# GATB/dsk

Measured on AMD Instinct MI355X. Metric: distinct k-mers counted/sec (whole node), k=31, higher is better.
Workload: dtype u64

## Files before the change

dsk_amd/csrc/dskgpu.hip:

```cpp
#include <algorithm>
#include <cstdio>
#include <cstring>
#include <cstdlib>
#include <cmath>
#include <string>
#include <vector>

#include <thread>
#include <system_error>
#include "engine.h"
#include "kernels.h"
#include "superkmer_recv.h"
#include "rawparse.h"

#include <rocprim/device/device_radix_sort.hpp>

#define DSKGPU_VERSION "dskgpu 0.1 (gfx950)"

namespace {

thread_local std::string g_create_err;

__global__ __launch_bounds__(1024) void k_place_probe(unsigned long long* __restrict__ out, unsigned long long n) {
    const unsigned long long per_block = n / gridDim.x, per_stream = per_block / 512;
    unsigned long long* base = out + (unsigned long long)blockIdx.x * per_block;
    const int r = threadIdx.x >> 5, l = threadIdx.x & 31;
    for (unsigned long long off = 0; off + 32 <= per_stream; off += 32)
        for (int p = r; p < 512; p += 32) base[(unsigned long long)p * per_stream + off + l] = off;
}
int g_place_k = -1;
float place_probe_ms(void* p, size_t bytes) {
    hipEvent_t a, b;
    if (hipEventCreate(&a) != hipSuccess || hipEventCreate(&b) != hipSuccess) return 0.f;
    float best = 1e30f;
    for (int i = 0; i < 3; ++i) {
        (void)hipEventRecord(a, 0);
        hipLaunchKernelGGL(k_place_probe, dim3(256), dim3(1024), 0, 0, static_cast<unsigned long long*>(p), (unsigned long long)(bytes / 8));
        (void)hipEventRecord(b, 0);
        (void)hipEventSynchronize(b);
        float ms = 0.f; (void)hipEventElapsedTime(&ms, a, b);
        if (i && ms < best) best = ms;
    }
    (void)hipEventDestroy(a); (void)hipEventDestroy(b);
    return best;
}
}

hipError_t placed_malloc(void** out, size_t bytes) {
    if (g_place_k < 0) { const char* e = getenv("DSKGPU_PLACE"); g_place_k = e ? atoi(e) : 0; }
    size_t free_b = 0, total_b = 0;
    if (g_place_k < 2 || bytes < (size_t(1) << 28) || hipMemGetInfo(&free_b, &total_b) != hipSuccess) return hipMalloc(out, bytes);
    const int K = (int)std::min<size_t>((size_t)g_place_k, free_b / 2 / bytes);
    if (K < 2) return hipMalloc(out, bytes);
    std::vector<void*> cand; std::vector<float> ms;
    for (int i = 0; i < K; ++i) {
        void* q = nullptr;
        if (hipMalloc(&q, bytes) != hipSuccess) { (void)hipGetLastError(); break; }
        static const size_t probe_max = getenv("DSKGPU_PLACE_GB") ? (size_t)(atof(getenv("DSKGPU_PLACE_GB")) * (1ull << 30)) : ~size_t(0);
        cand.push_back(q); ms.push_back(place_probe_ms(q, std::min(bytes, probe_max)));
    }
    if (cand.empty()) return hipErrorOutOfMemory;
    size_t best = 0;
    for (size_t i = 1; i < cand.size(); ++i) if (ms[i] < ms[best]) best = i;
    for (size_t i = 0; i < cand.size(); ++i) if (i != best) (void)hipFree(cand[i]);
// ... 194 lines not shown
template <int W>
inline void launch_count(dskgpu_ctx* ctx, unsigned grid, typename KeyT<W>::T* keys, typename KeyT<W>::T* solid_keys, u32* solid_ab, u32* ovf, const CountParams& cp) {
    launch_count_impl(ctx, grid, keys, solid_keys, solid_ab, ovf, cp);
}

struct Plan {
    int levels;
    u32 P1, P2, F;
    DigitSpec d1, d2;
};

#define TARGET_KEYS 2900
#define TARGET_KEYS2 2560
#ifndef TARGET_KEYS4
#define TARGET_KEYS4 640
#endif
#ifndef OPT_GROUPS4
#define OPT_GROUPS4 OPT_GROUPS
#endif
#define MAX_LEVEL_BINS 2048
#define ONE_LEVEL_BINS 1024
#define CH2 65536u
#define OPT_GROUPS 545u
#define OPT_GROUPS2 1023u
inline u32 opt_groups(int W) { return W == 2 ? (AL_G2 == 8 ? 1022u : OPT_GROUPS2) : (W == 1 && AL_G1 == 16) ? 546u : W == 4 ? OPT_GROUPS4 : OPT_GROUPS; }
inline u64 target_keys(int W) { return W == 1 ? TARGET_KEYS : W == 2 ? TARGET_KEYS2 : TARGET_KEYS4; }
#define OPT_CAP 4360u

bool make_plan(u64 n_upper, int extra_bits, int W, u32 num_cu, Plan* pl) {
    const u64 target = target_keys(W);
    u64 F = ((n_upper + target - 1) / target) << extra_bits;
    if (F < 2) F = 2;
    if (F <= ONE_LEVEL_BINS) { pl->levels = 1; pl->P1 = (u32)F; pl->P2 = 1; }
    else {
        u64 p2max = MAX_LEVEL_BINS; while (p2max > 64 && ascatter_lds(W, (u32)p2max) > 160 * 1024) --p2max;
        u64 p1 = 1; while (p1 * p1 < F) ++p1;
        const bool large = F >= (u64)num_cu * 64;
        if (large) {
            p1 = std::max<u64>((F + p2max - 2) / (p2max - 1), num_cu);
            p1 = (p1 + num_cu - 1) / num_cu * num_cu;
            if (p1 > MAX_LEVEL_BINS - 8) p1 = MAX_LEVEL_BINS - 8;
        }
        u64 p2 = (F + p1 - 1) / p1;
        if (p2 % 2 == 0 && p2 + 1 <= p2max) ++p2;
        if (p1 > MAX_LEVEL_BINS || p2 > MAX_LEVEL_BINS) return false;
        pl->levels = 2; pl->P1 = (u32)p1; pl->P2 = (u32)p2;
    }
    pl->F = pl->P1 * pl->P2;
    pl->d1 = DigitSpec{1u, pl->P1, 0u, 1u, 1u, 0u};
    pl->d2 = DigitSpec{2u, pl->P1, pl->P2, 1u, 1u, 0u};
    return true;
}

void build_descs1(dskgpu_ctx* ctx, u64 n_units_total, u64 tile, u64 max_chunks, u32* nch_out) {
    const u64 ntiles = std::max<u64>(1, (n_units_total + tile - 1) / tile);
    u64 nch = std::min<u64>(ntiles, max_chunks);
    const u64 tpc = (ntiles + nch - 1) / nch;
    nch = (ntiles + tpc - 1) / tpc;
    ctx->h_descs1.resize(nch);
    for (u64 c = 0; c < nch; ++c) {
        ChunkDesc d;
        d.begin = c * tpc * tile;
        d.end = std::min<u64>(n_units_total, (c + 1) * tpc * tile);
        if (d.begin > d.end) d.begin = d.end;
        d.flat_base = (u32)c;
        d.stride = (u32)nch;
        ctx->h_descs1[c] = d;
    }
    *nch_out = (u32)nch;
}

void build_descs1_slices(dskgpu_ctx* ctx, u64 tile, u64 max_chunks, u32* nch_out) {
    const size_t S = ctx->rec_slice_end.size();
    ctx->h_descs1.clear(); ctx->h_slice_chunk.assign(S + 1, 0);
    const u64 per_slice = std::max<u64>(1, max_chunks / S);
    u64 rb = 0;
    for (size_t sl = 0; sl < S; ++sl) {
        const u64 re = ctx->rec_slice_end[sl];
        ctx->h_slice_chunk[sl] = (u32)ctx->h_descs1.size();
        if (re > rb) {
            const u64 ntiles = (re - rb + tile - 1) / tile;
            u64 nch = std::min<u64>(ntiles, per_slice);
            const u64 tpc = (ntiles + nch - 1) / nch;
            nch = (ntiles + tpc - 1) / tpc;
            for (u64 c = 0; c < nch; ++c) {
                ChunkDesc d;
                d.begin = rb + c * tpc * tile; d.end = std::min<u64>(re, rb + (c + 1) * tpc * tile);
                d.flat_base = 0; d.stride = 0;
                ctx->h_descs1.push_back(d);
            }
        }
        rb = re;
    }
    ctx->h_slice_chunk[S] = (u32)ctx->h_descs1.size();
    for (auto& d : ctx->h_descs1) d.stride = (u32)ctx->h_descs1.size();
    *nch_out = (u32)ctx->h_descs1.size();
}

#define REC_RESIZE 1001
int rec_gate_upto(dskgpu_ctx* ctx, u32 upto) {
    if (!ctx->rec_gate) return DSKGPU_OK;
    const u32 n = (u32)ctx->rec_slice_end.size();
    for (; ctx->rec_gated < std::min(upto, n); ++ctx->rec_gated)
        if (ctx->rec_gate(ctx->rec_gate_user, ctx->rec_gated) != 0) ctx->rec_gate_failed = true;
    return ctx->rec_gate_failed ? fail(ctx, DSKGPU_E_STATE, "a slice of the exchange did not arrive (the caller's gate failed)") : DSKGPU_OK;
}
int rec_gate_all(dskgpu_ctx* ctx) { return rec_gate_upto(ctx, 0xFFFFFFFFu); }

int sk_sizes(dskgpu_ctx* ctx, u64* total_out) {
    const u64 nrec = ctx->rec_n; const u32 R = ctx->sender.sp.R;
    { const int e = rec_gate_all(ctx); if (e) return e; }
    u64 nch = std::min<u64>((nrec + SKX_NT - 1) / SKX_NT, (u64)ctx->num_cu * 16);
    u64 rpc = (nrec + nch - 1) / nch;
    rpc = (rpc + SKX_NT - 1) / SKX_NT * SKX_NT;
    nch = (nrec + rpc - 1) / rpc;
    if (rpc * SK_MAXN >= 0xFFFFFFFFull) return fail(ctx, DSKGPU_E_ARG, "too many records per chunk");
    CK(ctx->sk_sums.ensure(nch * 4)); CK(ctx->sk_cbase.ensure(nch * 8));
    ctx->h_sk_sums.assign(nch, 0); ctx->h_sk_cbase.assign(nch, 0);
    hipLaunchKernelGGL(k_sk_count, dim3((unsigned)nch), dim3(SKX_NT), 0, ctx->stream, ctx->rec_src, nrec, R, (u32)rpc, ctx->sk_sums.as<u32>());
    CKL("k_sk_count");
    CK(hipMemcpyAsync(ctx->h_sk_sums.data(), ctx->sk_sums.p, nch * 4, hipMemcpyDeviceToHost, ctx->stream));
    CK(hipStreamSynchronize(ctx->stream));
    u64 total = 0;
    for (u64 c = 0; c < nch; ++c) { ctx->h_sk_cbase[c] = total; total += ctx->h_sk_sums[c]; }
    CK(hipMemcpyAsync(ctx->sk_cbase.p, ctx->h_sk_cbase.data(), nch * 8, hipMemcpyHostToDevice, ctx->stream));
    ctx->rec_nch = nch; ctx->rec_rpc = rpc; ctx->rec_sized = true;
    *total_out = total;
    return DSKGPU_OK;
}

template <int W>
int expand_records(dskgpu_ctx* ctx, u64 total) {
    typedef typename KeyT<W>::T Key;
    if (ctx->rec_expanded) return DSKGPU_OK;
    if (!ctx->rec_sized) {
        u64 real = 0;
        const int e = sk_sizes(ctx, &real);
        if (e) return e;
        if (real != total && ctx->rec_hint_est) { ctx->rec_hint = real; return REC_RESIZE; }
        if (real != total) return fail(ctx, DSKGPU_E_ARG, "dskgpu_mg_count_sized: n_kmers does not match the k-mers inside the records");
    }
    { const int e = rec_gate_all(ctx); if (e) return e; }
    CK(ctx->sk_keys.ensure((total + 1) * sizeof(Key)));
    hipLaunchKernelGGL(k_sk_expand<W>, dim3((unsigned)ctx->rec_nch), dim3(SKX_NT), 0, ctx->stream, ctx->rec_src, ctx->rec_n, ctx->sender.sp.R,
                       (int)ctx->cfg.kmer_size, (u32)ctx->rec_rpc, ctx->sk_cbase.as<u64>(), ctx->sk_keys.as<Key>());
    CKL("k_sk_expand");
    ctx->rec_expanded = true;
    ctx->mark("mg_expand");
// ... 62 lines not shown
        u32 found = 0;
        for (u32 i = 0; i < n;) {
            u32 j = i + 1;
            while (j < n && kk[j] == kk[i]) ++j;
            if ((u64)(j - i) * 20 >= n) { cands.push_back({load[bin] * (double)(j - i) / (double)n, kk[i], bin}); ++found; }
            i = j;
        }
        if (ctx->tune.verbose) fprintf(stderr, "[dskgpu]   bin %u load %.0f: %u keys collected, %u dominant\n", bin, load[bin], n, found);
    }
    std::sort(cands.begin(), cands.end(), [](const Cand& a, const Cand& b) { return a.est > b.est; });
    if (cands.size() > HV_KEYS) cands.resize(HV_KEYS);
    ctx->h_hv_keys.assign((size_t)HV_KEYS * W, DSK_EMPTY);
    for (size_t x = 0; x < cands.size(); ++x) {
        for (int y = 0; y < W; ++y) ctx->h_hv_keys[x * W + y] = cands[x].key.w[y];
        load[cands[x].bin] -= cands[x].est;
    }
    u32 nheavy = (u32)cands.size();
    if (nheavy) {
        CK(ctx->hv_buf.ensure(HvLayout<W>::words * 8));
        u64* hvb = ctx->hv_buf.as<u64>();
        CK(hipMemsetAsync(hvb + HvLayout<W>::keys, 0xFF, (size_t)HV_KEYS * W * 8, ctx->stream));
        CK(hipMemsetAsync(hvb + HvLayout<W>::counts, 0, HV_KEYS * 8, ctx->stream));
        CK(hipMemcpyAsync(hvb + HvLayout<W>::keys, ctx->h_hv_keys.data(), (size_t)HV_KEYS * W * 8, hipMemcpyHostToDevice, ctx->stream));
    }
    *nheavy_out = nheavy;
    return DSKGPU_OK;
}

template <int W> struct KeySource { bool from_reads, from_rec; const typename KeyT<W>::T* keys; u64 nkeys, nwords; };

template <int W>
struct PassState {
    typedef typename KeyT<W>::T Key;
    KeySource<W>& src;
    u32 pass, npass; u64 cap;
    u64 nvalid;
    u32* sc;
    Plan pl{};
    u32 opt_cap = 0, max_ext = 0; u64 nregions = 0;
    bool opt1 = false; Opt1Spec o1{}; unsigned grid1 = 0;
    u32 nch1 = 0, nheavy = 0;
    std::vector<double> load, spread;
    Key* fkeys = nullptr;
    DevBuf* scratch = nullptr;
    Key* solid_keys = nullptr; u32* solid_ab = nullptr;
    u32 flags = 0, nsolid = 0, nkeys = 0, ovf2 = 0, ovf1 = 0, ext = 0; u64 stats[4] = {0, 0, 0, 0};
    bool too_big = false; u64 rows = 0;
};

template <int W>
int upload_descs1(dskgpu_ctx* ctx, PassState<W>& ps) {
    const KeySource<W>& src = ps.src;
    const u64 max_chunks1 = (u64)ctx->num_cu * 8;
    if (src.from_reads) build_descs1(ctx, src.nwords, Tile<W>::WORDS, max_chunks1, &ps.nch1);
    else if (src.from_rec && ctx->rec_slice_end.size() > 1) build_descs1_slices(ctx, RecTile<W>::NR, max_chunks1, &ps.nch1);
    else if (src.from_rec) build_descs1(ctx, ctx->rec_n, RecTile<W>::NR, max_chunks1, &ps.nch1);
    else build_descs1(ctx, src.nkeys, Tile<W>::KEYS, max_chunks1, &ps.nch1);
    CK(ctx->descs1.ensure(ctx->h_descs1.size() * sizeof(ChunkDesc)));
    CK(hipMemcpyAsync(ctx->descs1.p, ctx->h_descs1.data(), ctx->h_descs1.size() * sizeof(ChunkDesc), hipMemcpyHostToDevice, ctx->stream));
    return DSKGPU_OK;
}

template <int W>
int records_to_keys(dskgpu_ctx* ctx, PassState<W>& ps) {
    const int e = expand_records<W>(ctx, ps.src.nkeys);
    if (e) return e;
    ps.src.keys = ctx->sk_keys.template as<typename KeyT<W>::T>(); ps.src.from_rec = false;
    return upload_descs1(ctx, ps);
}

template <class Hist>
int positional_sample(dskgpu_ctx* ctx, u64 units, u64 tile, u32 P, Hist&& hist, u64* ntiles_out, u64* nts_out, u64* stot_out) {
    u32* sc = ctx->scalars.as<u32>();
    const u64 ntiles = std::max<u64>(1, (units + tile - 1) / tile);
    const u64 nts = std::min<u64>(ntiles, 1024);
    ctx->h_descs_s.resize(nts);
    for (u64 i = 0; i < nts; ++i) {
        const u64 t = i * ntiles / nts;
        ChunkDesc d; d.begin = t * tile; d.end = std::min<u64>(units, (t + 1) * tile); d.flat_base = (u32)i; d.stride = (u32)nts;
        ctx->h_descs_s[i] = d;
    }
    const u64 Ms = (u64)P * nts;
    CK(ctx->smp_descs.ensure(nts * sizeof(ChunkDesc)));
    CK(ctx->smp_mat.ensure((Ms + 4) * 4 + (size_t)P * 16));
    CK(hipMemcpyAsync(ctx->smp_descs.p, ctx->h_descs_s.data(), nts * sizeof(ChunkDesc), hipMemcpyHostToDevice, ctx->stream));
    ctx->h_sc[SC_NCH_S] = (u32)nts;
    CK(hipMemcpyAsync(sc + SC_NCH_S, &ctx->h_sc[SC_NCH_S], 4, hipMemcpyHostToDevice, ctx->stream));
    { const int e = hist(ctx->smp_descs.as<ChunkDesc>(), (const u32*)(sc + SC_NCH_S), nts, ctx->smp_mat.as<u32>()); if (e) return e; }
    u64* mom = reinterpret_cast<u64*>(ctx->smp_mat.as<u32>() + ((Ms + 2) & ~(u64)1));
    hipLaunchKernelGGL(k_bin_moments, dim3((P + 3) / 4), dim3(256), 0, ctx->stream, (const u32*)ctx->smp_mat.as<u32>(), (u32)nts, P, mom);
    CKL("k_bin_moments");
    ctx->h_mom.resize((size_t)P * 2);
    void* lz = landing(ctx, (size_t)P * 16);
    CK(hipMemcpyAsync(lz ? lz : (void*)ctx->h_mom.data(), mom, (size_t)P * 16, hipMemcpyDeviceToHost, ctx->stream));
    CK(hipStreamSynchronize(ctx->stream));
    if (lz) std::memcpy(ctx->h_mom.data(), lz, (size_t)P * 16);
    u64 stot = 0;
    for (u32 b = 0; b < P; ++b) stot += ctx->h_mom[2 * b];
    *ntiles_out = ntiles; *nts_out = nts; *stot_out = stot;
    return DSKGPU_OK;
}

template <int W>
int pass_plan(dskgpu_ctx* ctx, PassState<W>& ps, int extra_bits) {
    typedef typename KeyT<W>::T Key;
    Plan& pl = ps.pl;
    const u64 plan_n = (ps.src.from_reads && ctx->have_nvalid) ? std::min<u64>(ps.cap, ps.npass == 1 ? ps.nvalid + 1 : ps.nvalid / ps.npass + ps.nvalid / ps.npass / 50 + 4096) : ps.cap;
    if (!make_plan(plan_n, extra_bits, W, (u32)ctx->num_cu, &pl))
        return fail(ctx, DSKGPU_E_OVERFLOW, "cannot partition finer (table overflow persists)");
    pl.d1.world = pl.d2.world = ctx->cfg.world_size; pl.d1.npass = pl.d2.npass = ps.npass; pl.d1.pass = pl.d2.pass = ps.pass;
    { const int e = upload_descs1(ctx, ps); if (e) return e; }
    if (pl.levels == 2 && ctx->sentinel_ok && !ctx->opt2_off && !ctx->tune.no_opt2 && ascatter_lds(W, pl.P2) <= 160 * 1024)
        ps.opt_cap = opt_groups(W) * (8u / W);
    if (ps.opt_cap && ctx->tune.opt_cap) ps.opt_cap = ctx->tune.opt_cap;
    if (W > 1 && (u64)pl.F * ps.opt_cap >= 0xFFFF0000ull) ps.opt_cap = 0;
    const u32 opt_cap = ps.opt_cap;
    if (opt_cap && W <= 2) {
        u64 want = std::min<u64>((u64)pl.F / 8 + 4096, 0x7FFFFFFFull / opt_cap - 1);
        if (ctx->tune.max_ext >= 0) want = (u64)ctx->tune.max_ext;
        if (W > 1) { const u64 room = 0xFFFF0000ull / opt_cap; want = room > (u64)pl.F + 1 ? std::min<u64>(want, room - pl.F - 1) : 0; }
        ps.max_ext = (u32)want;
    }
    ps.nregions = (u64)pl.F + ps.max_ext;
    if (!opt_cap) { CK(ctx->bufA.ensure((ps.cap + 1) * sizeof(Key))); CK(ctx->bufB.ensure((ps.cap + 1) * sizeof(Key))); }
    if (opt_cap) {
        const u64 slots = (u64)pl.F * opt_cap + ATile<W>::KEYS + 16;
        CK(ctx->bufA.ensure(std::max<u64>(W == 1 ? slots * 4 : slots * sizeof(Key), (ps.cap + 1) * sizeof(Key))));
        if (W > 1) CK(ctx->abund2.ensure(slots * 4));
    }
    ps.opt1 = opt_cap && !ctx->opt1_off && !ctx->tune.no_opt1 && (ps.npass == 1 || ps.src.from_reads || W <= 2);
    if (ps.src.from_rec && (!ps.opt1 || W > 2 || ctx->tune.no_recsrc)) { const int e = records_to_keys(ctx, ps); if (e) return e; }
    if (ps.opt1 && scatter_lds(W, pl.P1, false) > 160 * 1024) ps.opt1 = false;
    return DSKGPU_OK;
}

template <int W>
int pass_layout1(dskgpu_ctx* ctx, PassState<W>& ps) {
    typedef typename KeyT<W>::T Key;
    const KeySource<W>& src = ps.src;
    const Plan& pl = ps.pl;
    Opt1Spec& o1 = ps.o1;
    o1 = Opt1Spec{nullptr, 0u, 0u, ps.sc + SC_OVF1, nullptr, ctx->sender.sp.R, ctx->gstats.as<u64>() + 2, nullptr, nullptr, 0u, nullptr, 0ull, {0ull, 0ull, 0ull, 0ull}, 0u};
    const bool uniform1 = scatter_lds(W, pl.P1, true) > 160 * 1024;
    if (ps.opt1) {
        const u32 nch1 = ps.nch1;
        const unsigned grid1 = ps.grid1 = scatter_grid(ctx, W, pl.P1, nch1, !uniform1);
        const u64 cpb = (nch1 + grid1 - 1) / grid1;
        double share = (double)cpb / (double)nch1;
        if (src.from_rec && ctx->rec_slice_end.size() > 1) {
            share = 0.0;
            u64 rb = 0;
            for (size_t sl = 0; sl < ctx->rec_slice_end.size(); ++sl) {
                const u64 re = ctx->rec_slice_end[sl], nc = ctx->h_slice_chunk[sl + 1] - ctx->h_slice_chunk[sl];
                if (nc) share += (double)((nc + grid1 - 1) / grid1) / (double)nc * (double)(re - rb) / (double)ctx->rec_n;
                rb = re;
            }
        }
        const double pass_keys = (double)(ps.nvalid / ps.npass);
        ps.load.assign(pl.P1, pass_keys / pl.P1);
        ps.spread.assign(pl.P1, 0.0);
        bool sampled = false;
        const Key* d_keys_s = src.keys;
        double smp_density = 1.0;
        bool rec_sample_ok = ctx->sentinel_ok;
        u64 rec_units = 0;
        if constexpr (W <= 2) {
          if (src.from_rec && !ctx->tune.no_sample && !uniform1) {
            const u64 nrec_s = ctx->rec_slice_end.size() > 1 ? ctx->rec_slice_end[0] : ctx->rec_n;
            const u64 NR = RecTile<W>::NR;
            const u64 nchk_all = (nrec_s + NR - 1) / NR;
            const u64 nchk = std::min<u64>(nchk_all, 256);
            if (nchk == 0) rec_sample_ok = false;
            else {
                { const int e = rec_gate_upto(ctx, 1); if (e) return e; }
                std::vector<u64>& cbeg = ctx->h_cbeg;
                cbeg.resize(nchk);
                for (u64 i = 0; i < nchk; ++i) cbeg[i] = (i * nchk_all / nchk) * NR;
                rec_units = nchk * NR * SK_MAXN;
                CK(ctx->smp_keys.ensure(rec_units * sizeof(Key) + nchk * 8 + 64));
                u64* d_cbeg = reinterpret_cast<u64*>(ctx->smp_keys.as<char>() + rec_units * sizeof(Key));
                CK(hipMemcpyAsync(d_cbeg, cbeg.data(), nchk * 8, hipMemcpyHostToDevice, ctx->stream));
                hipLaunchKernelGGL(k_sk_sample_keys<W>, dim3((unsigned)nchk), dim3(SKX_NT), 0, ctx->stream, ctx->rec_src, ctx->rec_n, ctx->sender.sp.R, (int)ctx->cfg.kmer_size,
                                   (const u64*)d_cbeg, (u32)NR, ctx->smp_keys.as<Key>());
                CKL("k_sk_sample_keys");
                d_keys_s = ctx->smp_keys.as<Key>();
            }
          }
        }
        const bool smp_rec = src.from_rec && rec_units != 0;
        if ((!src.from_rec || smp_rec) && rec_sample_ok && !ctx->tune.no_sample && !uniform1) {
            const u64 units = src.from_reads ? src.nwords : smp_rec ? rec_units : src.nkeys, tile = src.from_reads ? Tile<W>::WORDS : Tile<W>::KEYS;
            auto hist = [&](const ChunkDesc* dd, const u32* d_nch, u64 n, u32* mat) {
                return src.from_reads ? launch_hist<W, 0>(ctx, nullptr, dd, d_nch, n, mat, pl.d1, pl.P1) : launch_hist<W, 1>(ctx, d_keys_s, dd, d_nch, n, mat, pl.d1, pl.P1);
            };
            u64 ntiles = 0, nts = 0, stot = 0;
            { const int e = positional_sample(ctx, units, tile, pl.P1, hist, &ntiles, &nts, &stot); if (e) return e; }
            if (stot >= (u64)pl.P1 * 64) {
                const double scale = (src.from_reads && ps.npass > 1) ? (double)ntiles / (double)nts : pass_keys / (double)stot;
                if (smp_rec) smp_density = std::max(0.05, (double)stot / ((double)nts * (double)Tile<W>::KEYS));
                const double tiles_per_block = smp_rec ? pass_keys * share / (double)Tile<W>::KEYS : (double)ntiles * share;
                for (u32 b = 0; b < pl.P1; ++b) {
                    const double sum = (double)ctx->h_mom[2 * b], sq = (double)ctx->h_mom[2 * b + 1];
                    const double mean = sum / (double)nts, var = std::max(mean, sq / (double)nts - mean * mean);
                    ps.load[b] = sum * scale;
                    ps.spread[b] = 5.0 * std::sqrt(tiles_per_block * var / smp_density) + 4.0 * std::sqrt((double)nts * var) * scale * share;
                }
                sampled = true;
            }
            if constexpr (W <= 2) {
                if (sampled && ps.opt_cap && !ctx->tune.no_heavy) { const int e = find_heavy<W>(ctx, src.from_reads, d_keys_s, (u32)nts, pl, ps.load, &ps.nheavy); if (e) return e; }
// ... 337 lines not shown
    if (!sparse_sort && !mp_part) {
        hipLaunchKernelGGL(k_compact<W>, dim3((pl.F + 3) / 4), dim3(256), 0, ctx->stream, (const Key*)ps.solid_keys, (const u32*)ps.solid_ab,
                           ctx->fstart.as<u32>(), ctx->nsolid.as<u32>(), pl.F, ro, rows_ab, ps.opt_cap);
        CKL("k_compact");
    }
    ctx->mark("compact");
    ctx->stats.n_ext_regions += std::min<u32>(ps.ext, ps.max_ext);
    return DSKGPU_OK;
}

struct PassResult { u64 rows = 0, kmers = 0, distinct = 0, keys_seen = 0; Plan plan{}; bool too_big = false; };

template <int W>
int run_one_pass(dskgpu_ctx* ctx, bool from_reads, const typename KeyT<W>::T* d_keys_in, u64 nkeys_in, u64 nwords,
                 u32 pass, u32 npass, u64 cap, PassResult* res) {
    ctx->take_sparse_rows();
    KeySource<W> src{from_reads, !from_reads && d_keys_in == nullptr, d_keys_in, nkeys_in, nwords};
    const u64 nvalid = from_reads ? ctx->h_nvalid : nkeys_in;
    int extra_bits = 0, table_retries = 0;
    for (;;) {
        PassState<W> ps{src, pass, npass, cap, nvalid, ctx->scalars.as<u32>()};
        int e;
        if ((e = pass_plan<W>(ctx, ps, extra_bits)) || (e = pass_layout1<W>(ctx, ps)) || (e = pass_scatter1<W>(ctx, ps))) return e;
        if (ps.too_big) { ctx->resolve_marks(); res->too_big = true; res->keys_seen = ps.nkeys; return DSKGPU_OK; }
        if ((e = pass_scatter2<W>(ctx, ps)) || (e = pass_count<W>(ctx, ps))) return e;
        const bool ovf1 = ps.opt1 && ps.ovf1, ovf2 = ps.opt_cap && ps.ovf2;
        if (ovf1 || ovf2) {
            ctx->resolve_marks();
            if (ctx->tune.verbose) fprintf(stderr, "[dskgpu] pass %u/%u: %s overflowed: the exact path takes over\n", pass, npass, ovf1 ? "a level-1 slice" : "the level-2 extension pool");
            if (ovf1) ctx->opt1_off = true;
            else { ctx->opt2_off = true; ctx->opt1_off = true; }
            ctx->stats.n_retries += 1;
            ctx->mark("start");
            continue;
        }
        if (ps.flags & 1u) {
            ctx->resolve_marks();
            if (table_retries >= 3) return fail(ctx, DSKGPU_E_OVERFLOW, "hash table overflow after 3 retries");
            ++table_retries; extra_bits += 1;
            ctx->stats.n_retries += 1;
            ctx->mark("start");
            continue;
        }
        if ((e = pass_rows<W>(ctx, ps))) return e;
        res->rows = ps.rows; res->kmers = res->keys_seen = ps.nkeys; res->distinct = ps.stats[0]; res->plan = ps.pl;
        return DSKGPU_OK;
    }
}

int level0_materialise(dskgpu_ctx* ctx, u64 nwords, u32 lo, u32 npass, u64 reserve_bytes, u32* G_out, u64 (&region_keys)[L0_MAX_PASSES], u64 (&obase)[L0_MAX_PASSES]) {
    *G_out = 0;
    const u64 nper = ctx->h_nvalid / npass + 1;
    u32 nch1 = 0;
    build_descs1(ctx, nwords, Tile<1>::WORDS, (u64)ctx->num_cu * 8, &nch1);
    const unsigned grid = (unsigned)std::max<u64>(1, std::min<u64>(nch1, (u64)ctx->num_cu));
    const u64 cpb = (nch1 + grid - 1) / grid;
    const double share = (double)cpb / (double)nch1;
    const u64 tail = 2 * Tile<1>::KEYS;
    const u64 uslice = (((u64)((double)nper * share * 1.02) + 4096) + 7) & ~7ull;
    const u64 uregion = uslice * grid + tail;
    if (uregion >= 0xFFFF0000ull) return DSKGPU_OK;
    size_t free_b = 0, total_b = 0;
    CK(hipMemGetInfo(&free_b, &total_b));
    const u64 have = ctx->bufA.cap + ctx->bufB.cap + ctx->l0buf.cap;
    const u64 need = nper * 30ull + (4ull << 30) + reserve_bytes;
    const u64 room = free_b + have > need ? free_b + have - need : 0;
    u32 G = (u32)std::min<u64>(std::min<u64>(L0_MAX_PASSES, npass - lo), room / (uregion * 8));
    if (ctx->tune.l0_passes) G = std::min<u32>(std::min<u32>(ctx->tune.l0_passes, L0_MAX_PASSES), npass - lo);
    if (G < 2 && !(ctx->tune.l0_passes)) return DSKGPU_OK;
    if (G == 0) return DSKGPU_OK;
    CK(ctx->descs1.ensure(ctx->h_descs1.size() * sizeof(ChunkDesc)));
    CK(hipMemcpyAsync(ctx->descs1.p, ctx->h_descs1.data(), ctx->h_descs1.size() * sizeof(ChunkDesc), hipMemcpyHostToDevice, ctx->stream));
    u32* sc = ctx->scalars.as<u32>();
    DigitSpec ds{4u, G, 0u, ctx->cfg.world_size, npass, lo};
    std::vector<u64> slice(G, uslice);
    if (!ctx->tune.no_sample) {
        auto hist = [&](const ChunkDesc* dd, const u32* d_nch, u64 n, u32* mat) { return launch_hist_m<1, 0, 4>(ctx, nullptr, dd, d_nch, n, mat, ds, G); };
        u64 ntiles = 0, nts = 0, stot = 0;
        { const int e = positional_sample(ctx, nwords, Tile<1>::WORDS, G, hist, &ntiles, &nts, &stot); if (e) return e; }
        if (stot >= (u64)G * 4096) {
            const double scale = (double)ntiles / (double)nts, tiles_per_block = (double)ntiles * share;
            for (u32 b = 0; b < G; ++b) {
                const double sum = (double)ctx->h_mom[2 * b], sq = (double)ctx->h_mom[2 * b + 1];
                const double mean = sum / (double)nts, var = std::max(mean, sq / (double)nts - mean * mean);
                const double sl = sum * scale * share * 1.01 + 5.0 * std::sqrt(tiles_per_block * var) + 4.0 * std::sqrt((double)nts * var) * scale * share + 64.0;
                slice[b] = ((u64)sl + 8) & ~7ull;
            }
        }
        ctx->mark("sample0");
    }
    for (;;) {
        u64 tot = 0; bool ok = true;
        for (u32 b = 0; b < G; ++b) { const u64 region = slice[b] * grid + tail; if (region >= 0xFFFF0000ull) ok = false; obase[b] = tot; region_keys[b] = slice[b] * grid; tot += region; }
        if (ok && (tot * 8 <= room || ctx->tune.l0_passes)) { CK(ctx->l0buf.ensure(tot * 8 + 64)); break; }
        if (--G < 2) return DSKGPU_OK;
    }
    ds.pa = G;
    ctx->h_sc[SC_NCH1] = nch1; ctx->h_sc[SC_OVF1] = 0;
    CK(hipMemcpyAsync(sc + SC_NCH1, &ctx->h_sc[SC_NCH1], 4, hipMemcpyHostToDevice, ctx->stream));
    CK(hipMemsetAsync(sc + SC_OVF1, 0, 4, ctx->stream));
    ctx->h_boff.assign(L0_MAX_PASSES + 1 + 3 + 2 * L0_MAX_PASSES, 0);
    u64 hob[L0_MAX_PASSES];
    for (u32 i = 0; i < L0_MAX_PASSES; ++i) { ctx->h_boff[i] = (u32)slice[std::min(i, G - 1)]; hob[i] = obase[std::min(i, G - 1)]; }
    std::memcpy(&ctx->h_boff[L0_MAX_PASSES + 4], hob, sizeof hob);
    CK(ctx->boff.ensure(ctx->h_boff.size() * 4));
    CK(hipMemcpyAsync(ctx->boff.p, ctx->h_boff.data(), ctx->h_boff.size() * 4, hipMemcpyHostToDevice, ctx->stream));
    const u32* d_slen = ctx->boff.as<u32>();
    const u64* d_obase = reinterpret_cast<const u64*>(ctx->boff.as<u32>() + L0_MAX_PASSES + 4);
    hipLaunchKernelGGL(k_level0, dim3(grid), dim3(SC_NT), 0, ctx->stream, (const u64*)ctx->packed.as<u64>(), (const u32*)ctx->inval.as<u32>(), (const ChunkDesc*)ctx->descs1.as<ChunkDesc>(),
                       (const u32*)(sc + SC_NCH1), ctx->l0buf.as<u64>(), (int)ctx->cfg.kmer_size, ds, G, d_slen, d_obase, sc + SC_OVF1);
// ... 174 lines not shown
                for (size_t i = 0; i < pass_hist.size(); ++i) ctx->hist[i] += pass_hist[i];
                ctx->resolve_marks();
                ctx->mark("start");
            }
            tot_rows += ns;
        }
        if (rec_l0) { ctx->sender.prepared = false; ctx->enc_fresh = false; }
        if (restart) {
            ctx->rec_l0_off = true;
            ctx->resolve_marks();
            return run_pipeline<W>(ctx, from_reads, d_keys_in, nkeys_in);
        }
        if (too_big) {
            if (seen + (1u << 20) < 0xFFFF0000ull && seen > cap_floor) cap_floor = seen + (1u << 20); else { npass *= 2; cap_floor = 0; }
            continue;
        }
        if (npass > 1) {
            std::swap(ctx->out_ab, ctx->acc_ab);
            for (int x = 0; x < W; ++x) std::swap(ctx->out_w[x], ctx->acc_w[x]);
        }
        if (const int rc = order_rows(ctx, tot_rows, npass)) return rc;
        ctx->resolve_marks();
        ctx->n_rows = tot_rows;
        ctx->stats.n_bytes = from_reads ? ctx->n_bytes : 0;
        ctx->stats.n_kmers = tot_kmers;
        ctx->stats.n_distinct = tot_distinct;
        ctx->stats.n_solid = tot_rows;
        ctx->stats.n_levels = (u32)pl.levels;
        ctx->stats.n_final_bins = pl.F;
        ctx->stats.n_passes = npass;
        ctx->stats.n_read_sweeps = npass > 1 ? sweeps : (from_reads ? 1 : 0);
        if (from_reads) ctx->last_rows = tot_rows;
        if (npass > 1) {
            std::swap(ctx->out_ab, ctx->acc_ab);
            for (int x = 0; x < W; ++x) std::swap(ctx->out_w[x], ctx->acc_w[x]);
        }
        ctx->stats.n_partitions = rows_partitions(ctx);
        ctx->have_result = true;
        return DSKGPU_OK;
    }
}

template <int W>
int mg_scatter_impl(dskgpu_ctx* ctx, void* d_send, uint64_t* send_words) {
    typedef typename KeyT<W>::T Key;
    ctx->st_names.clear(); ctx->st_ms.clear(); ctx->marks.clear(); ctx->ev_used = 0;
    ctx->mark("start");
    u64 nwords = 0;
    int rc = encode_current(ctx, &nwords);
    if (rc) return rc;
    ctx->mark("encode");
    const u32 G = ctx->cfg.world_size;
    u32 nch1 = 0;
    build_descs1(ctx, nwords, Tile<W>::WORDS, (u64)ctx->num_cu * 8, &nch1);
    const u64 M1 = (u64)G * nch1;
    CK(ctx->scalars.ensure(SC_COUNT * 4));
    CK(ctx->descs1.ensure(ctx->h_descs1.size() * sizeof(ChunkDesc)));
    CK(hipMemcpyAsync(ctx->descs1.p, ctx->h_descs1.data(), ctx->h_descs1.size() * sizeof(ChunkDesc), hipMemcpyHostToDevice, ctx->stream));
    u32* h_sc = ctx->h_sc;
    std::memset(h_sc, 0, sizeof(ctx->h_sc));
    h_sc[SC_NCH1] = nch1; h_sc[SC_MLEN1] = (u32)M1;
    u32* sc = ctx->scalars.as<u32>();
    CK(hipMemcpyAsync(sc, h_sc, sizeof(ctx->h_sc), hipMemcpyHostToDevice, ctx->stream));
    CK(ctx->mat1.ensure((M1 + 1) * 4));
    const DigitSpec owner = DigitSpec{0u, G, 0u, G, 1u, 0u};
    if ((rc = launch_hist<W, 0>(ctx, nullptr, ctx->descs1.as<ChunkDesc>(), sc + SC_NCH1, nch1, ctx->mat1.as<u32>(), owner, G))) return rc;
    ctx->mark("mg_hist");
    if ((rc = run_scan(ctx, ctx->mat1.as<u32>(), sc + SC_MLEN1, M1))) return rc;
    if ((rc = launch_scatter<W, 0>(ctx, nullptr, ctx->descs1.as<ChunkDesc>(), sc + SC_NCH1, nch1, ctx->mat1.as<u32>(), static_cast<Key*>(d_send), owner, G))) return rc;
    ctx->mark("mg_scatter");
    ctx->h_starts.assign(G + 1, 0);
    for (u32 o = 0; o <= G; ++o)
        CK(hipMemcpyAsync(&ctx->h_starts[o], ctx->mat1.as<u32>() + (u64)o * nch1, 4, hipMemcpyDeviceToHost, ctx->stream));
    CK(hipStreamSynchronize(ctx->stream));
    ctx->resolve_marks();
    for (u32 o = 0; o < G; ++o) send_words[o] = (u64)(ctx->h_starts[o + 1] - ctx->h_starts[o]) * W;
    return DSKGPU_OK;
}

template <int W>
int sk_count(dskgpu_ctx* ctx, const u64* d_rec, u64 recv_words, u64 n_kmers_hint, bool hint_is_estimate = false) {
    typedef typename KeyT<W>::T Key;
    const u32 R = ctx->sender.sp.R;
    if (recv_words % R) return fail(ctx, DSKGPU_E_ARG, "recv_words is not a whole number of super-k-mer records");
    const u64 nrec = recv_words / R;
    if (hint_is_estimate && ctx->marks.size() > 1) {
        CK(hipStreamSynchronize(ctx->stream));
        ctx->resolve_marks();
    }
    ctx->marks.clear(); ctx->ev_used = 0;
    ctx->mark("start");
    u64 total = 0;
    ctx->rec_hint = 0; ctx->rec_sized = false; ctx->rec_hint_est = hint_is_estimate;
    if (nrec) {
        ctx->rec_src = d_rec; ctx->rec_n = nrec; ctx->rec_expanded = false;
        if (n_kmers_hint) { total = n_kmers_hint; ctx->rec_hint = n_kmers_hint; }
        else { const int e = sk_sizes(ctx, &total); if (e) return e; }
    } else {
        ctx->rec_src = nullptr; ctx->rec_n = 0;
        CK(ctx->sk_keys.ensure(sizeof(Key)));
    }
    ctx->mark("mg_sizes");
    CK(hipStreamSynchronize(ctx->stream));
    ctx->resolve_marks();
    if (!ctx->rec_src) { const int e = rec_gate_all(ctx); if (e) return e; return run_pipeline<W>(ctx, false, ctx->sk_keys.as<Key>(), 0); }
    int rc = run_pipeline<W>(ctx, false, nullptr, total);
    if (rc == REC_RESIZE) { ctx->rec_hint_est = false; rc = run_pipeline<W>(ctx, false, nullptr, ctx->rec_hint); ctx->rec_hint = 0; }
// ... 724 lines not shown
```

dsk_amd/csrc/kernels.h:

```cpp
#pragma once
#include "layouts.h"

#ifndef SC_NT
#define SC_NT 1024
#endif
template <int W> struct Tile {
    static constexpr int KPT = 16 / W;
    static constexpr int KEYS = SC_NT * KPT;
    static constexpr int WORDS = KEYS / 32;
};
#define MAX_BINS 2048


template <bool ALIGNED>
__global__ __launch_bounds__(256) void k_encode(const uint8_t* __restrict__ s, u64 n,
                                                u64* __restrict__ packed, u32* __restrict__ inval, u64 nwords) {
    const u64 stride = (u64)gridDim.x * blockDim.x;
    for (u64 w = (u64)blockIdx.x * blockDim.x + threadIdx.x; w < nwords; w += stride) {
        const u64 base = w * 32;
        u32 x[8];
        if (ALIGNED && base + 32 <= n) {
            const uint4 a = *reinterpret_cast<const uint4*>(s + base);
            const uint4 b = *reinterpret_cast<const uint4*>(s + base + 16);
            x[0] = a.x; x[1] = a.y; x[2] = a.z; x[3] = a.w; x[4] = b.x; x[5] = b.y; x[6] = b.z; x[7] = b.w;
// ... 375 lines not shown
    if (OPT && o1.uslice) for (u32 b = threadIdx.x; b < P; b += SC_NT) cur[b] = first + b * o1.uslice;
    else if (OPT && MODE == 4) for (u32 b = threadIdx.x; b < P; b += SC_NT) { const u32 sl = o1.boff[b]; cur[b] = blockIdx.x * sl; lim[b] = cur[b] + sl; lob[b] = o1.obase[b]; }
    else if (OPT) for (u32 b = threadIdx.x; b < P; b += SC_NT) { cur[b] = first + o1.boff[b]; lim[b] = first + o1.boff[b + 1]; }
    u32 gbeg = blockIdx.x, gend = nchunks;
    if constexpr (SRC == 2 && OPT) {
        if (o1.cur_state) { gbeg += o1.g0; gend = o1.g0 + o1.gn; }
        if (o1.resume) for (u32 b = threadIdx.x; b < P; b += SC_NT) cur[b] = o1.cur_state[(u64)blockIdx.x * P + b];
    }
    Key hvk[HV_KEYS]; u32 hc[HV_KEYS]; int nhk = 0;
    if constexpr (HEAVY) {
#pragma unroll
        for (int x = 0; x < HV_KEYS; ++x) { hvk[x] = reinterpret_cast<const Key*>(o1.hv_keys)[x]; hc[x] = 0; if (!is_empty_key(hvk[x])) nhk = x + 1; }
    }
    for (u32 g = gbeg; g < gend; g += gridDim.x) {
        const ChunkDesc d = descs[g];
        lds_barrier();
        for (u32 b = threadIdx.x; b < P; b += SC_NT) { if (!OPT) cur[b] = scanned[d.flat_base + (u64)b * d.stride]; cnt[b] = 0; }
        if (threadIdx.x == 0) cnt[P] = 0;
        const u64 step = SRC == 0 ? Tile<W>::WORDS : Tile<W>::KEYS;
        Key ha[KPT], hb[KPT]; u32 vma = 0, vmb = 0;
        auto rank_and_stage = [&](Key (&h)[KPT], u32 vm) {
            if constexpr (HEAVY && W <= 2) {
#pragma unroll
                for (int x = 0; x < HV_KEYS; ++x) {
                    if (x < nhk) {
                        u32 hits = 0;
#pragma unroll
                        for (int j = 0; j < KPT; ++j) hits |= keys_same(h[j], hvk[x]) ? (1u << j) : 0u;
                        hits &= vm;
                        hc[x] += (u32)__popc(hits);
                        vm &= ~hits;
                    }
                }
            }
            u32 rk[KPT];
#pragma unroll
            for (int j = 0; j < KPT; ++j) {
                u32 dj = key_digit<MODE>(digit_word(h[j]), ds);
                asm volatile("" : "+v"(dj));
                dj = ((vm & (1u << j)) && key_in_pass<MODE>(digit_word(h[j]), ds)) ? dj : P;
                rk[j] = dj << 16;
            }
#pragma unroll
            for (int j = 0; j < KPT; ++j) if ((rk[j] >> 16) < P) rk[j] |= atomicAdd(&cnt[rk[j] >> 16], 1u);
            lds_barrier();
            tile_scan<SC_NT>(cnt, off, delta, cur, (int)P, wsum, tot, OPT ? SliceGuard{o1.uslice ? nullptr : lim, o1.dump, o1.uslice, first} : SliceGuard{nullptr, 0u, 0u, 0u});
            lds_barrier();
#pragma unroll
            for (int j = 0; j < KPT; ++j) if ((rk[j] >> 16) < P) stage[off[rk[j] >> 16] + (rk[j] & 0xFFFFu)] = h[j];
            lds_barrier();
        };
        auto write_out = [&]() {
            const u32 ntile = *tot;
#pragma unroll
            for (int it = 0; it < (KPT + 3) / 4; ++it) {
                const u32 i0 = (u32)it * 4 * SC_NT;
                if constexpr (W >= 4) {
#pragma unroll
                    for (int u = 0; u < 4; ++u) {
                        const u32 i = i0 + u * SC_NT + threadIdx.x;
                        const Key kv = stage[i];
                        const u32 dg = key_digit<MODE>(digit_word(kv), ds);
                        const u32 d1 = delta[MODE == 4 ? (dg < P ? dg : 0u) : dg];
                        if (OPT) out[i < ntile ? (u64)(d1 + i) : (u64)(o1.dump + i)] = kv;
                        else if (i < ntile) out[(u64)(d1 + i)] = kv;
                    }
                    continue;
                }
                Key hk[4]; u32 dd[4];
#pragma unroll
                for (int u = 0; u < 4; ++u) hk[u] = stage[i0 + u * SC_NT + threadIdx.x];
#pragma unroll
                for (int u = 0; u < 4; ++u) {
                    const u32 dg = key_digit<MODE>(digit_word(hk[u]), ds);
                    dd[u] = delta[MODE == 4 ? (dg < P ? dg : 0u) : dg];
                }
#pragma unroll
                for (int u = 0; u < 4; ++u) {
                    const u32 i = i0 + u * SC_NT + threadIdx.x;
                    if (OPT && MODE == 4) out[i < ntile ? lob[key_digit<MODE>(digit_word(hk[u]), ds) & (L0_MAX_PASSES - 1)] + (u64)(dd[u] + i) : o1.obase0 + (u64)(o1.dump + i)] = hk[u];
                    else if (OPT) out[i < ntile ? (u64)(dd[u] + i) : (u64)(o1.dump + i)] = hk[u];
                    else if (i < ntile) out[(u64)(dd[u] + i)] = hk[u];
                }
            }
        };
        auto process = [&](Key (&h)[KPT], u32 vm) { rank_and_stage(h, vm); write_out(); };
        if (SRC == 1 && d.begin < d.end) vma = tile_keys_array<W>(keys, d.begin, d.end, ha);
        lds_barrier();
        if constexpr (SRC == 2) {
            if constexpr (W <= 2) {
                RecPre<W> pre;
                if (d.begin < d.end) rec_prefetch<W>(pre, packed, o1.R, d.begin, d.end);
                for (u64 r0 = d.begin; r0 < d.end;) {
                    u32 taken = 0;
                    vma = tile_keys_records<W>(pre, o1.R, r0, d.end, k, ha, smem, wsum, &taken);
                    rank_and_stage(ha, vma);
                    r0 += taken ? taken : 1u;
                    if (r0 < d.end) rec_prefetch<W>(pre, packed, o1.R, r0, d.end);
                    write_out();
                }
            }
        } else if constexpr (SRC == 0 && W == 1) {
            struct Raw { u64 cur, prev; u32 ic, ip; };
            const u32 wlane = threadIdx.x & (SC_NT / 2 - 1);
            const bool upper = threadIdx.x >= SC_NT / 2;
            auto load_raw = [&](u64 t0) {
                const u64 wi = t0 + wlane;
                const u64 wc = wi < d.end ? wi : d.end - 1;
                Raw r; r.cur = packed[wc]; r.prev = packed[wc ? wc - 1 : 0]; r.ic = inval[wc]; r.ip = inval[wc ? wc - 1 : 0];
                if (wc == 0) { r.prev = 0ull; r.ip = 0xFFFFFFFFu; }
                return r;
            };
            if (d.begin < d.end) {
                Raw raw = load_raw(d.begin);
                if (OPT) {
                    u64* dz = out + (MODE == 4 ? o1.obase0 : 0ull) + (u64)(o1.dump + threadIdx.x);
                    asm volatile("" : "+v"(dz));
#pragma unroll
                    for (int u = 0; u < 4 * ((KPT + 3) / 4); ++u) dz[u * SC_NT] = (u64)threadIdx.x;
                }
                for (u64 t0 = d.begin; t0 < d.end; t0 += step) {
                    const bool live = t0 + wlane < d.end;
                    if (upper) vma = gen_kmers1_words<16>(raw.cur, raw.prev, raw.ic, raw.ip, 16, k, ha);
                    else vma = gen_kmers1_words<16>(raw.cur, raw.prev, raw.ic, raw.ip, 0, k, ha);
                    if (!live) vma = 0u;
#pragma unroll
                    for (int j = 0; j < 16; ++j) ha[j] = kmix(ha[j]);
                    rank_and_stage(ha, vma);
                    const u64 tn = t0 + step < d.end ? t0 + step : t0;
                    raw = load_raw(tn);
                    write_out();
                }
            }
        } else if constexpr (SRC == 0 && W == 2) {
            struct Raw2 { u64 cur, p1, p2; u32 ic, i1, i2; };
            const u32 wlane = threadIdx.x & (SC_NT / 4 - 1);
            const u32 quarter = threadIdx.x / (SC_NT / 4);
            auto load_raw = [&](u64 t0) {
                const u64 wi = t0 + wlane;
                const u64 wc = wi < d.end ? wi : d.end - 1;
                Raw2 r; r.cur = packed[wc]; r.p1 = packed[wc >= 1 ? wc - 1 : 0]; r.p2 = packed[wc >= 2 ? wc - 2 : 0];
                r.ic = inval[wc]; r.i1 = inval[wc >= 1 ? wc - 1 : 0]; r.i2 = inval[wc >= 2 ? wc - 2 : 0];
                if (wc < 1) { r.p1 = 0ull; r.i1 = 0xFFFFFFFFu; }
                if (wc < 2) { r.p2 = 0ull; r.i2 = 0xFFFFFFFFu; }
                return r;
            };
            if (d.begin < d.end) {
                Raw2 raw = load_raw(d.begin);
                if (OPT) {
                    Key fillk; fillk.w[0] = fillk.w[1] = (u64)threadIdx.x;
#pragma unroll
                    for (int u = 0; u < 4 * ((KPT + 3) / 4); ++u) out[(u64)(o1.dump + u * SC_NT + threadIdx.x)] = fillk;
                }
                for (u64 t0 = d.begin; t0 < d.end; t0 += step) {
                    const bool live = t0 + wlane < d.end;
                    if (quarter == 0) vma = gen_kmers2_words<8>(raw.cur, raw.p1, raw.p2, raw.ic, raw.i1, raw.i2, 0, k, ha);
                    else if (quarter == 1) vma = gen_kmers2_words<8>(raw.cur, raw.p1, raw.p2, raw.ic, raw.i1, raw.i2, 8, k, ha);
                    else if (quarter == 2) vma = gen_kmers2_words<8>(raw.cur, raw.p1, raw.p2, raw.ic, raw.i1, raw.i2, 16, k, ha);
                    else vma = gen_kmers2_words<8>(raw.cur, raw.p1, raw.p2, raw.ic, raw.i1, raw.i2, 24, k, ha);
                    if (!live) vma = 0u;
#pragma unroll
                    for (int j = 0; j < 8; ++j) kmixN(ha[j]);
                    rank_and_stage(ha, vma);
                    const u64 tn = t0 + step < d.end ? t0 + step : t0;
                    raw = load_raw(tn);
                    write_out();
                }
            }
        } else if constexpr (SRC == 0) {
            for (u64 t0 = d.begin; t0 < d.end; t0 += step) {
                vma = tile_keys_reads(packed, inval, t0, d.end, k, ha);
                process(ha, vma);
            }
        } else {
            for (u64 t0 = d.begin; t0 < d.end; t0 += 2 * step) {
                if (t0 + step < d.end) vmb = tile_keys_array<W>(keys, t0 + step, d.end, hb);
                process(ha, vma);
                const u64 t1 = t0 + step;
                if (t1 >= d.end) break;
                if (t1 + step < d.end) vma = tile_keys_array<W>(keys, t1 + step, d.end, ha);
                process(hb, vmb);
            }
        }
    }
    if (OPT) {
        lds_barrier();
        if constexpr (HEAVY) {
#pragma unroll
            for (int x = 0; x < HV_KEYS; ++x) {
                u32 v = hc[x];
#pragma unroll
                for (int dd = 32; dd >= 1; dd >>= 1) v += __shfl_down(v, dd);
                if ((threadIdx.x & 63) == 0 && v) atomicAdd(&o1.hv_cnt[x], (unsigned long long)v);
            }
        }
        if constexpr (SRC == 2) {
            if (o1.cur_state) {
                for (u32 b = threadIdx.x; b < P; b += SC_NT) o1.cur_state[(u64)blockIdx.x * P + b] = cur[b];
                if (!o1.last) return;
            }
        }
        bool ovf = false;
        u32 mine = 0;
        for (u32 b = threadIdx.x; b < P; b += SC_NT) {
            const u32 beg = MODE == 4 ? blockIdx.x * o1.boff[b] : first + (o1.uslice ? b * o1.uslice : o1.boff[b]), c = cur[b], end = o1.uslice ? beg + o1.uslice : lim[b];
// ... 1537 lines not shown
```

Before: 27.09 billion.

## Balance stage-1 chunks across scatter grid and shrink per-lane dump slots

Chunk descriptors are now built so that chunks are dealt round-robin across the actual scatter grid, with tile counts spread evenly per block and per round. The per-block share estimate is computed from the real busiest block instead of a ceiling formula. The goal is less tail imbalance between blocks and a tighter output slice reservation. Separately, the dump area for dead lanes collapses to one slot per lane (for SRC != 1), which shrinks dump memory and the warm-up writes. The catch is more host-side descriptor logic, and dead lanes now write repeatedly to the same address.

```diff
diff --git a/dsk_amd/csrc/chunks1.h b/dsk_amd/csrc/chunks1.h
--- /dev/null
+++ b/dsk_amd/csrc/chunks1.h
@@ -0,0 +1,66 @@
+#pragma once
+#include <algorithm>
+#include <cstddef>
+#include <cstdint>
+#include <vector>
+
+template <class Desc>
+inline void chunks1_append(std::vector<Desc>& out, uint64_t base, uint64_t n_units, uint64_t tile, uint64_t max_chunks, uint64_t grid_cap) {
+    const uint64_t ntiles = std::max<uint64_t>(1, (n_units + tile - 1) / tile);
+    const uint64_t nmax = std::max<uint64_t>(1, std::min<uint64_t>(ntiles, max_chunks));
+    const uint64_t grid = std::max<uint64_t>(1, std::min<uint64_t>(nmax, grid_cap));
+    const uint64_t rounds = nmax / grid;
+    const uint64_t q = ntiles / grid, rem = ntiles % grid;
+    uint64_t t = 0;
+    for (uint64_t r = 0; r < rounds; ++r)
+        for (uint64_t b = 0; b < grid; ++b) {
+            const uint64_t mine = q + (b < rem ? 1 : 0);
+            const uint64_t len = mine / rounds + (r < mine % rounds ? 1 : 0);
+            Desc d{};
+            d.begin = base + std::min<uint64_t>(n_units, t * tile);
+            d.end = base + std::min<uint64_t>(n_units, (t + len) * tile);
+            out.push_back(d);
+            t += len;
+        }
+}
+
+template <class Desc, class U64>
+inline void chunks1_build(std::vector<Desc>& out, std::vector<uint32_t>& slice_chunk, const std::vector<U64>& slice_end, uint64_t tile,
+                          uint64_t max_chunks, uint64_t grid_cap) {
+    const size_t S = slice_end.size();
+    out.clear(); slice_chunk.assign(S + 1, 0);
+    const uint64_t per_slice = S > 1 ? std::max<uint64_t>(grid_cap, max_chunks / S) : max_chunks;
+    uint64_t rb = 0;
+    for (size_t sl = 0; sl < S; ++sl) {
+        const uint64_t re = slice_end[sl];
+        slice_chunk[sl] = (uint32_t)out.size();
+        if (re > rb || S == 1) chunks1_append(out, rb, re - rb, tile, per_slice, grid_cap);
+        rb = re;
+    }
+    slice_chunk[S] = (uint32_t)out.size();
+}
+
+template <class Desc>
+inline uint64_t chunks1_busiest_tiles(const Desc* d, size_t n, uint64_t grid, uint64_t tile) {
+    uint64_t best = 0;
+    for (uint64_t b = 0; b < grid && b < n; ++b) {
+        uint64_t s = 0;
+        for (size_t c = b; c < n; c += grid) s += (d[c].end - d[c].begin + tile - 1) / tile;
+        best = std::max(best, s);
+    }
+    return best;
+}
+template <class Desc>
+inline uint64_t chunks1_tiles(const Desc* d, size_t n, uint64_t tile) {
+    uint64_t s = 0;
+    for (size_t c = 0; c < n; ++c) s += (d[c].end - d[c].begin + tile - 1) / tile;
+    return s;
+}
+template <class Desc>
+inline double chunks1_share(const std::vector<Desc>& d, const std::vector<uint32_t>& slice_chunk, uint64_t grid, uint64_t tile) {
+    uint64_t busiest = 0;
+    for (size_t s = 0; s + 1 < slice_chunk.size(); ++s)
+        busiest += chunks1_busiest_tiles(d.data() + slice_chunk[s], slice_chunk[s + 1] - slice_chunk[s], grid, tile);
+    const uint64_t all = chunks1_tiles(d.data(), d.size(), tile);
+    return all ? (double)busiest / (double)all : 1.0;
+}
diff --git a/dsk_amd/csrc/dskgpu.hip b/dsk_amd/csrc/dskgpu.hip
--- a/dsk_amd/csrc/dskgpu.hip
+++ b/dsk_amd/csrc/dskgpu.hip
@@ -10,6 +10,7 @@
 #include <system_error>
 #include "engine.h"
 #include "kernels.h"
+#include "chunks1.h"
 #include "superkmer_recv.h"
 #include "rawparse.h"
 
@@ -310,48 +311,16 @@
     return true;
 }
 
-void build_descs1(dskgpu_ctx* ctx, u64 n_units_total, u64 tile, u64 max_chunks, u32* nch_out) {
-    const u64 ntiles = std::max<u64>(1, (n_units_total + tile - 1) / tile);
-    u64 nch = std::min<u64>(ntiles, max_chunks);
-    const u64 tpc = (ntiles + nch - 1) / nch;
-    nch = (ntiles + tpc - 1) / tpc;
-    ctx->h_descs1.resize(nch);
-    for (u64 c = 0; c < nch; ++c) {
-        ChunkDesc d;
-        d.begin = c * tpc * tile;
-        d.end = std::min<u64>(n_units_total, (c + 1) * tpc * tile);
-        if (d.begin > d.end) d.begin = d.end;
-        d.flat_base = (u32)c;
-        d.stride = (u32)nch;
-        ctx->h_descs1[c] = d;
-    }
-    *nch_out = (u32)nch;
-}
-
-void build_descs1_slices(dskgpu_ctx* ctx, u64 tile, u64 max_chunks, u32* nch_out) {
-    const size_t S = ctx->rec_slice_end.size();
-    ctx->h_descs1.clear(); ctx->h_slice_chunk.assign(S + 1, 0);
-    const u64 per_slice = std::max<u64>(1, max_chunks / S);
-    u64 rb = 0;
-    for (size_t sl = 0; sl < S; ++sl) {
-        const u64 re = ctx->rec_slice_end[sl];
-        ctx->h_slice_chunk[sl] = (u32)ctx->h_descs1.size();
-        if (re > rb) {
-            const u64 ntiles = (re - rb + tile - 1) / tile;
-            u64 nch = std::min<u64>(ntiles, per_slice);
-            const u64 tpc = (ntiles + nch - 1) / nch;
-            nch = (ntiles + tpc - 1) / tpc;
-            for (u64 c = 0; c < nch; ++c) {
-                ChunkDesc d;
-                d.begin = rb + c * tpc * tile; d.end = std::min<u64>(re, rb + (c + 1) * tpc * tile);
-                d.flat_base = 0; d.stride = 0;
-                ctx->h_descs1.push_back(d);
-            }
-        }
-        rb = re;
-    }
-    ctx->h_slice_chunk[S] = (u32)ctx->h_descs1.size();
-    for (auto& d : ctx->h_descs1) d.stride = (u32)ctx->h_descs1.size();
+void build_descs1(dskgpu_ctx* ctx, u64 n_units_total, u64 tile, u64 max_chunks, u64 grid_cap, u32* nch_out) {
+    chunks1_build(ctx->h_descs1, ctx->h_slice_chunk, std::vector<u64>{n_units_total}, tile, max_chunks, grid_cap);
+    u32 c = 0;
+    for (auto& d : ctx->h_descs1) { d.flat_base = c++; d.stride = (u32)ctx->h_descs1.size(); }
+    *nch_out = (u32)ctx->h_descs1.size();
+}
+
+void build_descs1_slices(dskgpu_ctx* ctx, u64 tile, u64 max_chunks, u64 grid_cap, u32* nch_out) {
+    chunks1_build(ctx->h_descs1, ctx->h_slice_chunk, ctx->rec_slice_end, tile, max_chunks, grid_cap);
+    for (auto& d : ctx->h_descs1) { d.flat_base = 0; d.stride = (u32)ctx->h_descs1.size(); }
     *nch_out = (u32)ctx->h_descs1.size();
 }
 
@@ -520,10 +489,11 @@
 int upload_descs1(dskgpu_ctx* ctx, PassState<W>& ps) {
     const KeySource<W>& src = ps.src;
     const u64 max_chunks1 = (u64)ctx->num_cu * 8;
-    if (src.from_reads) build_descs1(ctx, src.nwords, Tile<W>::WORDS, max_chunks1, &ps.nch1);
-    else if (src.from_rec && ctx->rec_slice_end.size() > 1) build_descs1_slices(ctx, RecTile<W>::NR, max_chunks1, &ps.nch1);
-    else if (src.from_rec) build_descs1(ctx, ctx->rec_n, RecTile<W>::NR, max_chunks1, &ps.nch1);
-    else build_descs1(ctx, src.nkeys, Tile<W>::KEYS, max_chunks1, &ps.nch1);
+    const u64 grid_cap = scatter_grid(ctx, W, ps.pl.P1, max_chunks1, scatter_lds(W, ps.pl.P1, true) <= 160 * 1024);
+    if (src.from_reads) build_descs1(ctx, src.nwords, Tile<W>::WORDS, max_chunks1, grid_cap, &ps.nch1);
+    else if (src.from_rec && ctx->rec_slice_end.size() > 1) build_descs1_slices(ctx, RecTile<W>::NR, max_chunks1, grid_cap, &ps.nch1);
+    else if (src.from_rec) build_descs1(ctx, ctx->rec_n, RecTile<W>::NR, max_chunks1, grid_cap, &ps.nch1);
+    else build_descs1(ctx, src.nkeys, Tile<W>::KEYS, max_chunks1, grid_cap, &ps.nch1);
     CK(ctx->descs1.ensure(ctx->h_descs1.size() * sizeof(ChunkDesc)));
     CK(hipMemcpyAsync(ctx->descs1.p, ctx->h_descs1.data(), ctx->h_descs1.size() * sizeof(ChunkDesc), hipMemcpyHostToDevice, ctx->stream));
     return DSKGPU_OK;
@@ -613,17 +583,8 @@
     if (ps.opt1) {
         const u32 nch1 = ps.nch1;
         const unsigned grid1 = ps.grid1 = scatter_grid(ctx, W, pl.P1, nch1, !uniform1);
-        const u64 cpb = (nch1 + grid1 - 1) / grid1;
-        double share = (double)cpb / (double)nch1;
-        if (src.from_rec && ctx->rec_slice_end.size() > 1) {
-            share = 0.0;
-            u64 rb = 0;
-            for (size_t sl = 0; sl < ctx->rec_slice_end.size(); ++sl) {
-                const u64 re = ctx->rec_slice_end[sl], nc = ctx->h_slice_chunk[sl + 1] - ctx->h_slice_chunk[sl];
-                if (nc) share += (double)((nc + grid1 - 1) / grid1) / (double)nc * (double)(re - rb) / (double)ctx->rec_n;
-                rb = re;
-            }
-        }
+        const u64 tile1 = src.from_reads ? Tile<W>::WORDS : src.from_rec ? RecTile<W>::NR : Tile<W>::KEYS;
+        const double share = chunks1_share(ctx->h_descs1, ctx->h_slice_chunk, grid1, tile1);
         const double pass_keys = (double)(ps.nvalid / ps.npass);
         ps.load.assign(pl.P1, pass_keys / pl.P1);
         ps.spread.assign(pl.P1, 0.0);
@@ -1067,10 +1028,9 @@
     *G_out = 0;
     const u64 nper = ctx->h_nvalid / npass + 1;
     u32 nch1 = 0;
-    build_descs1(ctx, nwords, Tile<1>::WORDS, (u64)ctx->num_cu * 8, &nch1);
+    build_descs1(ctx, nwords, Tile<1>::WORDS, (u64)ctx->num_cu * 8, (u64)ctx->num_cu, &nch1);
     const unsigned grid = (unsigned)std::max<u64>(1, std::min<u64>(nch1, (u64)ctx->num_cu));
-    const u64 cpb = (nch1 + grid - 1) / grid;
-    const double share = (double)cpb / (double)nch1;
+    const double share = chunks1_share(ctx->h_descs1, ctx->h_slice_chunk, grid, Tile<1>::WORDS);
     const u64 tail = 2 * Tile<1>::KEYS;
     const u64 uslice = (((u64)((double)nper * share * 1.02) + 4096) + 7) & ~7ull;
     const u64 uregion = uslice * grid + tail;
@@ -1351,7 +1311,7 @@
     ctx->mark("encode");
     const u32 G = ctx->cfg.world_size;
     u32 nch1 = 0;
-    build_descs1(ctx, nwords, Tile<W>::WORDS, (u64)ctx->num_cu * 8, &nch1);
+    build_descs1(ctx, nwords, Tile<W>::WORDS, (u64)ctx->num_cu * 8, scatter_grid(ctx, W, G, (u64)ctx->num_cu * 8), &nch1);
     const u64 M1 = (u64)G * nch1;
     CK(ctx->scalars.ensure(SC_COUNT * 4));
     CK(ctx->descs1.ensure(ctx->h_descs1.size() * sizeof(ChunkDesc)));
diff --git a/dsk_amd/csrc/kernels.h b/dsk_amd/csrc/kernels.h
--- a/dsk_amd/csrc/kernels.h
+++ b/dsk_amd/csrc/kernels.h
@@ -451,6 +451,8 @@
         };
         auto write_out = [&]() {
             const u32 ntile = *tot;
+            constexpr bool LANE_SLOT = SRC != 1;
+            auto slot = [&](bool live, u32 dl, u32 i, u32 first) { return LANE_SLOT ? (u64)(i + (live ? dl : o1.dump - first)) : live ? (u64)(dl + i) : (u64)(o1.dump + i); };
 #pragma unroll
             for (int it = 0; it < (KPT + 3) / 4; ++it) {
                 const u32 i0 = (u32)it * 4 * SC_NT;
@@ -461,7 +463,7 @@
                         const Key kv = stage[i];
                         const u32 dg = key_digit<MODE>(digit_word(kv), ds);
                         const u32 d1 = delta[MODE == 4 ? (dg < P ? dg : 0u) : dg];
-                        if (OPT) out[i < ntile ? (u64)(d1 + i) : (u64)(o1.dump + i)] = kv;
+                        if (OPT) out[slot(i < ntile, d1, i, i0 + u * SC_NT)] = kv;
                         else if (i < ntile) out[(u64)(d1 + i)] = kv;
                     }
                     continue;
@@ -477,8 +479,8 @@
 #pragma unroll
                 for (int u = 0; u < 4; ++u) {
                     const u32 i = i0 + u * SC_NT + threadIdx.x;
-                    if (OPT && MODE == 4) out[i < ntile ? lob[key_digit<MODE>(digit_word(hk[u]), ds) & (L0_MAX_PASSES - 1)] + (u64)(dd[u] + i) : o1.obase0 + (u64)(o1.dump + i)] = hk[u];
-                    else if (OPT) out[i < ntile ? (u64)(dd[u] + i) : (u64)(o1.dump + i)] = hk[u];
+                    if (OPT && MODE == 4) out[i < ntile ? lob[key_digit<MODE>(digit_word(hk[u]), ds) & (L0_MAX_PASSES - 1)] + (u64)(dd[u] + i) : o1.obase0 + slot(false, 0u, i, i0 + u * SC_NT)] = hk[u];
+                    else if (OPT) out[slot(i < ntile, dd[u], i, i0 + u * SC_NT)] = hk[u];
                     else if (i < ntile) out[(u64)(dd[u] + i)] = hk[u];
                 }
             }
@@ -516,7 +518,7 @@
                     u64* dz = out + (MODE == 4 ? o1.obase0 : 0ull) + (u64)(o1.dump + threadIdx.x);
                     asm volatile("" : "+v"(dz));
 #pragma unroll
-                    for (int u = 0; u < 4 * ((KPT + 3) / 4); ++u) dz[u * SC_NT] = (u64)threadIdx.x;
+                    for (int u = 0; u < 4 * ((KPT + 3) / 4); ++u) { dz[0] = (u64)threadIdx.x; asm volatile("" : "+v"(dz)); }
                 }
                 for (u64 t0 = d.begin; t0 < d.end; t0 += step) {
                     const bool live = t0 + wlane < d.end;
@@ -548,8 +550,9 @@
                 Raw2 raw = load_raw(d.begin);
                 if (OPT) {
                     Key fillk; fillk.w[0] = fillk.w[1] = (u64)threadIdx.x;
-#pragma unroll
-                    for (int u = 0; u < 4 * ((KPT + 3) / 4); ++u) out[(u64)(o1.dump + u * SC_NT + threadIdx.x)] = fillk;
+                    u32 dz = o1.dump + threadIdx.x;
+#pragma unroll
+                    for (int u = 0; u < 4 * ((KPT + 3) / 4); ++u) { asm volatile("" : "+v"(dz)); out[(u64)dz] = fillk; }
                 }
                 for (u64 t0 = d.begin; t0 < d.end; t0 += step) {
                     const bool live = t0 + wlane < d.end;
```

Result: no change. 26.95 billion (-0.5%).
